# AaltoML/free-hunch

Measured on AMD Instinct MI355X. Metric: images/sec (256x256, num_steps=30, FH-Heun), higher is better.
Workload: dtype f32 UNet (convolutions: exact 3-way bf16 split on the bf16 MFMA, fp32 accuracy) + f64 covariance/CG; 1 GPU; FFHQ-256 arch, gaussian_blur, FH low-rank covariance (dct_diagonal), num_steps=30 heun, batch=8 per GPU; lockstep_groups_per_gpu=2, unet_backend=hip, net_calls_per_image=59

## Files before the change

### free-hunch_amd/_lib.py

```python
from __future__ import annotations

import ctypes as C
import os

import torch

_HERE = os.path.dirname(os.path.abspath(__file__))
LIB_PATH = os.path.join(_HERE, "libfh_hip.so")

c_dp = C.c_void_p


class FhProblem(C.Structure):
    _fields_ = [("op", C.c_int32), ("use_dct", C.c_int32), ("planes", C.c_int32), ("stride", C.c_int32),
                ("ntaps", C.c_int32), ("m", C.c_int32), ("ldm", C.c_int32), ("halo", C.c_int32),
                ("d", C.c_int64), ("sigma_y2", C.c_double),
                ("tap_dy", c_dp), ("tap_dx", c_dp), ("tap_w", c_dp), ("mask", c_dp),
                ("D", c_dp), ("r", c_dp), ("B", c_dp), ("M", c_dp),
                ("ntaps2", C.c_int32), ("halo2", C.c_int32), ("cg_scipy", C.c_int32), ("fold_sym", C.c_int32),
                ("tap2_dy", c_dp), ("tap2_dx", c_dp), ("tap2_w", c_dp),
                ("fold_fwd_w", c_dp), ("fold_fwd_h", c_dp), ("fold_inv_w", c_dp), ("fold_inv_h", c_dp)]


FH_MAX_BATCH = 16
# ... 12 lines not shown


class FhGnEpilogue(C.Structure):
    _fields_ = [("partial", c_dp), ("x", c_dp), ("tab", c_dp), ("mode", C.c_int32), ("act", C.c_int32), ("in_amax", c_dp)]


class FhCgInfo(C.Structure):
    _fields_ = [("niter", C.c_int32), ("optimal", C.c_int32), ("residual_norm", C.c_double),
                ("b_norm", C.c_double)]


_SIGS = {
    "fh_version": ([], C.c_int),
    "fh_context_create": ([C.POINTER(C.c_void_p), C.c_int, C.c_int, C.c_int], C.c_int),
    "fh_context_destroy": ([C.c_void_p], C.c_int),
    "fh_context_set_exclusive": ([C.c_void_p, C.c_int], C.c_int),
    "fh_context_status": ([C.c_void_p, C.c_void_p], C.c_int),
    "fh_debug_read_stamps": ([C.c_void_p, C.POINTER(C.c_ulonglong), C.c_int, C.c_void_p], C.c_int),
    "fh_dct2d": ([C.c_void_p, c_dp, c_dp, C.c_int, C.c_int, C.c_void_p], C.c_int),
    "fh_dct_moments_u8": ([C.c_void_p, c_dp, C.c_int, c_dp, c_dp, c_dp, C.c_void_p], C.c_int),
    "fh_rep_apply": ([C.c_void_p, c_dp, c_dp, c_dp, c_dp, C.c_int, c_dp, c_dp, C.c_int64, C.c_int, C.c_void_p], C.c_int),
    "fh_rep_apply_batched": ([C.c_void_p, C.POINTER(FhBatch), C.c_int, c_dp, c_dp, C.c_int64, C.c_int, C.c_void_p], C.c_int),
    "fh_rep_invert": ([C.c_void_p, c_dp, c_dp, c_dp, C.c_double, c_dp, c_dp, c_dp, C.c_int, C.c_int64, C.c_int,
                       C.c_void_p], C.c_int),
    "fh_space_prep": ([C.c_void_p, c_dp, C.c_double, c_dp, c_dp, c_dp, C.c_int64, C.c_void_p], C.c_int),
    "fh_dot": ([C.c_void_p, c_dp, c_dp, c_dp, C.c_int, C.c_int64, C.c_void_p], C.c_int),
    "fh_space_commit": ([C.c_void_p, c_dp, c_dp, C.c_double, C.c_double, C.c_double, c_dp, c_dp, c_dp, c_dp, c_dp,
                         c_dp, c_dp, c_dp, C.c_int, C.c_int64, C.c_void_p], C.c_int),
    "fh_space_commit_dev": ([C.c_void_p, c_dp, c_dp, c_dp, C.c_double, c_dp, c_dp, c_dp, c_dp, c_dp, c_dp, c_dp, c_dp,
                             c_dp, C.c_int, C.c_int, c_dp, C.c_int, C.c_int, C.c_int, C.c_int64, C.c_void_p], C.c_int),
    "fh_cov_time_update": ([C.c_void_p, C.POINTER(FhCovState), c_dp, c_dp, C.c_double, C.c_double, C.c_double, C.c_int,
                            c_dp, c_dp, c_dp, c_dp, C.c_void_p], C.c_int),
    "fh_cov_space_update": ([C.c_void_p, C.POINTER(FhCovState), c_dp, c_dp, C.c_double, c_dp, c_dp, C.c_void_p], C.c_int),
    "fh_cov_time_update_batched": ([C.c_void_p, C.c_int, C.POINTER(FhCovState), c_dp, c_dp, C.c_double, C.c_double, C.c_double,
                                    c_dp, c_dp, c_dp, C.c_void_p], C.c_int),
    "fh_cov_space_update_batched": ([C.c_void_p, C.c_int, C.POINTER(FhCovState), c_dp, c_dp, C.c_double, c_dp, c_dp, c_dp,
                                     C.c_void_p], C.c_int),
    "fh_woodbury_inner": ([C.c_void_p, c_dp, C.c_int, c_dp, C.c_int, c_dp, C.c_int, C.c_int, C.c_void_p], C.c_int),
    "fh_axpby": ([C.c_double, c_dp, C.c_double, c_dp, c_dp, C.c_int64, C.c_void_p], C.c_int),
    "fh_read_scalars": ([C.c_void_p, c_dp, C.POINTER(C.c_double), C.c_int, C.c_void_p], C.c_int),
    "fh_conv_circ": ([C.c_void_p, c_dp, c_dp, c_dp, c_dp, c_dp, C.c_int, C.c_int, C.c_int, C.c_int, C.c_int,
                      C.c_void_p], C.c_int),
    "fh_channel_mix": ([C.c_void_p, c_dp, c_dp, c_dp, C.c_int, C.c_int, C.c_void_p], C.c_int),
    "fh_amm": ([C.c_void_p, C.POINTER(FhProblem), c_dp, c_dp, C.c_void_p], C.c_int),
    "fh_dense_matvec_scratch_doubles": ([C.c_int, C.c_int64], C.c_int64),
    "fh_dense_matvec": ([c_dp, c_dp, c_dp, c_dp, C.c_int, C.c_int64, C.c_int, C.c_double, C.c_double, C.c_void_p], C.c_int),
    "fh_dense_rank2": ([c_dp, c_dp, C.c_int, C.c_int64, c_dp, c_dp, c_dp, c_dp, c_dp, c_dp, C.c_double, C.c_double,
                        C.c_void_p], C.c_int),
    "fh_conv2d_nhwc": ([c_dp, c_dp, c_dp, c_dp, c_dp, c_dp] + [C.c_int] * 10 + [C.c_void_p], C.c_int),
    "fh_conv2d_x6_nhwc": ([c_dp, c_dp, c_dp, c_dp, c_dp, c_dp] + [C.c_int] * 10 + [C.c_void_p], C.c_int),
    "fh_conv2d_x6_nhwc_gn": ([c_dp, c_dp, c_dp, c_dp, c_dp, c_dp] + [C.c_int] * 10 + [C.POINTER(FhGnEpilogue), C.c_void_p],
                             C.c_int),
    "fh_conv2d_x6_gn_chunks": ([C.c_int] * 10, C.c_int),
    "fh_groupnorm_finalize": ([c_dp, c_dp, C.c_int, C.c_int, C.c_double, C.c_int, C.c_void_p], C.c_int),
    "fh_groupnorm_bwd_table": ([c_dp, c_dp, c_dp, c_dp, c_dp, C.c_int, c_dp, C.c_int, C.c_int, C.c_void_p], C.c_int),
    "fh_groupnorm_bwd_apply": ([c_dp] * 8 + [C.c_int, c_dp] + [C.c_int] * 5 + [C.c_void_p], C.c_int),
    "fh_groupnorm_bwd_sums": ([c_dp] * 7 + [C.c_int, c_dp, c_dp] + [C.c_int] * 4 + [C.c_void_p], C.c_int),
    "fh_groupnorm_bwd_apply_ex": ([c_dp] * 8 + [C.c_int, c_dp, c_dp, c_dp, c_dp] + [C.c_int] * 5 + [c_dp, C.c_void_p], C.c_int),
    "fh_conv2d_splitk": ([C.c_int] * 7, C.c_int),
    "fh_unet_set_precision": ([C.c_int], C.c_int),
    "fh_unet_get_precision": ([], C.c_int),
    "fh_absmax_f32": ([c_dp, C.c_int64, c_dp, C.c_void_p], C.c_int),
    "fh_groupnorm_table": ([c_dp, c_dp, c_dp, c_dp, c_dp, C.c_int, c_dp, C.c_int, C.c_int, C.c_void_p], C.c_int),
    "fh_conv2d_x6_norm_supported": ([C.c_int] * 5, C.c_int),
    "fh_conv2d_x6_norm_nhwc": ([c_dp, c_dp, C.c_int, c_dp, c_dp, c_dp, c_dp] + [C.c_int] * 5 + [C.c_void_p], C.c_int),
    "fh_conv2d_x6_norm_nhwc_gn": ([c_dp, c_dp, C.c_int, c_dp, c_dp, c_dp, c_dp] + [C.c_int] * 5
                                  + [C.POINTER(FhGnEpilogue), C.c_void_p], C.c_int),
    "fh_conv3x3_thin_nhwc": ([c_dp, c_dp, c_dp, c_dp] + [C.c_int] * 5 + [C.c_void_p], C.c_int),
    "fh_conv3x3_wino_nhwc": ([c_dp, c_dp, c_dp, c_dp, c_dp] + [C.c_int] * 5 + [C.c_void_p], C.c_int),
    "fh_bgemm_f32": ([c_dp, c_dp, c_dp] + [C.c_int] * 10 + [C.c_int64] * 6 + [C.c_float, C.c_void_p], C.c_int),
    "fh_groupnorm_scratch_doubles": ([C.c_int, C.c_int], C.c_int64),
    "fh_groupnorm_stats": ([c_dp, c_dp, c_dp, C.c_int, C.c_int, C.c_int, C.c_void_p], C.c_int),
    "fh_groupnorm_apply": ([c_dp] * 6 + [C.c_int, c_dp, C.c_int, C.c_int, C.c_int, C.c_int, C.c_void_p], C.c_int),
    "fh_groupnorm_bwd": ([c_dp] * 7 + [C.c_int, c_dp, c_dp, c_dp] + [C.c_int] * 5 + [C.c_void_p], C.c_int),
    "fh_attention_supported": ([C.c_int] * 3, C.c_int),
    "fh_attention_fwd": ([c_dp, c_dp, c_dp] + [C.c_int] * 5 + [C.c_void_p], C.c_int),
    "fh_attention_bwd": ([c_dp] * 6 + [C.c_int] * 5 + [C.c_void_p], C.c_int),
    "fh_softmax_rows": ([c_dp, C.c_int64, C.c_int, C.c_void_p], C.c_int),
    "fh_softmax_bwd_rows": ([c_dp, c_dp, C.c_int64, C.c_int, C.c_void_p], C.c_int),
    "fh_resample2x": ([c_dp, c_dp] + [C.c_int] * 5 + [C.c_void_p], C.c_int),
    "fh_concat_channels": ([c_dp, c_dp, c_dp, C.c_int64, C.c_int, C.c_int, C.c_int, C.c_void_p], C.c_int),
    "fh_layout_nchw_nhwc": ([c_dp, c_dp, C.c_int, C.c_int, C.c_int64, C.c_int, C.c_int, C.c_void_p], C.c_int),
    "fh_add_f32": ([c_dp, c_dp, c_dp, C.c_int64, C.c_void_p], C.c_int),
    "fh_metrics_scratch_doubles": ([C.c_int] * 4, C.c_int64),
    "fh_metrics_u8": ([c_dp, c_dp, C.c_int, C.c_int, C.c_int, C.c_int, c_dp, c_dp, c_dp, C.c_void_p], C.c_int),
    "fh_lpips_prep_u8": ([c_dp, c_dp, c_dp, c_dp, C.c_int, C.c_int, C.c_int, C.c_void_p], C.c_int),
    "fh_relu_f32": ([c_dp, C.c_int64, C.c_void_p], C.c_int),
    "fh_relu_maxpool2_nhwc": ([c_dp, c_dp, C.c_int, C.c_int, C.c_int, C.c_int, C.c_void_p], C.c_int),
    "fh_lpips_tap_scratch_doubles": ([C.c_int], C.c_int64),
    "fh_lpips_tap": ([c_dp, c_dp, C.c_int, C.c_int, C.c_int, C.c_int, c_dp, c_dp, C.c_int, C.c_void_p], C.c_int),
    "fh_cg_solve_batched": ([C.c_void_p, C.POINTER(FhProblem), C.POINTER(FhBatch), c_dp, c_dp, C.POINTER(C.c_double),
                             C.c_double, C.c_int, C.POINTER(FhCgInfo), C.c_void_p], C.c_int),
    "fh_cg_solve": ([C.c_void_p, C.POINTER(FhProblem), c_dp, c_dp, C.c_double, C.c_double, C.c_int,
                     C.POINTER(FhCgInfo), C.c_void_p], C.c_int),
}

_lib = None


class FhError(RuntimeError):
    pass


def load():
    global _lib
    if _lib is None:
# ... 102 lines not shown
```

### free-hunch_amd/csrc/fh_unet.hip

```cpp
#include "fh_common.h"
#include <stdlib.h>

typedef float float16_t __attribute__((ext_vector_type(16)));

namespace {

constexpr int kBK = 32;
constexpr int kLd = kBK + 4;

struct ConvArgs {
  const float* in;
  const float* w;
  const float* bias;
  const float* res;
  float* out;
  int N, H, W, Cin, Cout, KH, KW, pad, stride, Ho, Wo;
  int ksplit;
  float* ws;
};

__device__ __forceinline__ void xcd_tile(int& tile_m, int& tile_n) {
  const unsigned gx = gridDim.x, gy = gridDim.y;
  const unsigned total = gx * gy;
  unsigned lin = blockIdx.y * gx + blockIdx.x;
// ... 412 lines not shown
    float tb[5] = {0.f, 0.f, 0.f, 0.f, 0.f};
    if (gn && a.gn_mode == 1) {
#pragma unroll
      for (int q = 0; q < 5; ++q) tb[q] = a.gn_tab[((int64_t)gn_n * 5 + q) * a.Cout + co];
    }
#pragma unroll
    for (int i = 0; i < MI; ++i) {
#pragma unroll
      for (int r = 0; r < 16; ++r) {
        const int64_t row = m0 + wm + i * 32 + (r & 3) + 8 * (r >> 2) + 4 * lh;
        if (row < M) {
          float v = acc[i][j][r];
          if (F16 && NP == 2) v = v * ssc.inv_in * ssc.winv;
          v += bv;
          if (a.res != nullptr && a.ksplit == 1) v += a.res[row * a.Cout + co];
          dst[row * a.Cout + co] = v;
          if (gn) gn_accum(a, gsum[j], v, row, co, tb);
        }
      }
    }
  }
  if (gn) {
    const int tiles_per_img = (int)(((int64_t)a.Ho * a.Wo) / BM);
    gn_reduce<NI, WM, WN, BN>(a, gsum, gred, gn_n, (tile_m % tiles_per_img) * (int)gridDim.y + tile_n, n0);
  }
}

template <int SEGW, bool NORM = false, int BM = 128, int NP = 3, int GL = 0, bool F16 = false>
__global__ __launch_bounds__(4 * BM, 4) void k_conv_x6r(ConvArgsX a) {
  constexpr int MI = 2, NI = 1, WN = 4, T = 4 * BM;
  constexpr int NSEG = BM / SEGW, SP = SEGW + 2;
  constexpr int BN = 128, AR = NSEG * SP;
  constexpr int IA = (AR * 8 + T - 1) / T;
  constexpr int IB = (NP * BN * 4 + T - 1) / T;
  constexpr int NB = GL == 2 ? 3 : (GL ? 2 : 1);
  constexpr int NA = GL == 2 ? 2 : 1;
  static_assert(GL != 2 || (NP * 8 == T / 64), "deep pipeline: one weight DMA per wave and tap");
  constexpr int BLD = GL ? kBK : kXLd;
  constexpr int kAsBytes = NA * NP * AR * kXLd * 2, kBsBytes = NB * NP * BN * BLD * 2;
  constexpr int kGredBytes = (BM / 64) * WN * 32 * NI * 2 * 8;
  __shared__ __align__(16) unsigned char smem[kAsBytes + kBsBytes + kGredBytes];
  __bf16 (*As)[NP][AR][kXLd] = reinterpret_cast<__bf16 (*)[NP][AR][kXLd]>(smem);
  __bf16 (*Bs)[NP][BN][BLD] = reinterpret_cast<__bf16 (*)[NP][BN][BLD]>(smem + kAsBytes);
  double* gred = reinterpret_cast<double*>(smem + kAsBytes + kBsBytes);
  const int tid = threadIdx.x, lane = tid & 63, wave = tid >> 6;
  const int wm = (wave / WN) * (MI * 32), wn = (wave % WN) * (NI * 32);
  const int lr = lane & 31, lh = lane >> 5;
  int tile_m, tile_n;
  xcd_tile(tile_m, tile_n);
  const int64_t m0 = (int64_t)tile_m * BM;
  const int n0 = tile_n * BN;
  const int cpt = a.Cin / kBK;
  const int nchunks = cpt * 9;
  const int pn = (int)(m0 / ((int64_t)a.H * a.W));
  const int rem = (int)(m0 % ((int64_t)a.H * a.W));
  const int py = rem / a.W, px0 = rem % a.W;

  int a_row[IA], a_seg[IA], a_gx[IA];
  bool a_in[IA];
  const int a_c4 = (tid & 7) * 4;
#pragma unroll
  for (int e = 0; e < IA; ++e) {
    const int idx = e * T + tid;
    a_row[e] = idx >> 3;
    a_seg[e] = a_row[e] / SP;
    a_gx[e] = px0 - 1 + a_row[e] % SP;
    a_in[e] = idx < AR * 8 && a_gx[e] >= 0 && a_gx[e] < a.W;
    if (idx >= AR * 8) a_row[e] = -1;
  }
  const int64_t wplane = (int64_t)9 * cpt * a.Cout * kBK;
  const SplitScale ssc = split_scale<NP, F16>(a, wplane);
  int b_pl[IB], b_row[IB];
  bool b_ok[IB];
  const int b_part = (tid & 3) * 8;
#pragma unroll
  for (int e = 0; e < IB; ++e) {
    const int idx = e * T + tid;
    b_pl[e] = idx < NP * BN * 4 ? idx / (BN * 4) : -1;
    b_row[e] = (idx % (BN * 4)) >> 2;
    b_ok[e] = b_pl[e] >= 0 && n0 + b_row[e] < a.Cout;
  }
  float4 ra_reg[IA];
  bool ra_ok[IA];
  float4 tA = make_float4(1.f, 1.f, 1.f, 1.f), tB = make_float4(0.f, 0.f, 0.f, 0.f);
  bf16x8_t rb_reg[IB];
  auto load_a = [&](int cc, int ky) {
    if (NORM) {
      const float* t = a.ab + (int64_t)pn * 2 * a.Cin + cc * kBK + a_c4;
      tA = *reinterpret_cast<const float4*>(t);
      tB = *reinterpret_cast<const float4*>(t + a.Cin);
    }
    const float* base = a.in + (int64_t)pn * a.H * a.W * a.Cin + cc * kBK + a_c4;
#pragma unroll
    for (int e = 0; e < IA; ++e) {
      const int gy = py + a_seg[e] + ky - 1;
      const bool ok = a_in[e] && gy >= 0 && gy < a.H;
      ra_ok[e] = ok;
      if (GL == 2) {
        const float4 v = *reinterpret_cast<const float4*>(base + ((int64_t)(ok ? gy : 0) * a.W + (ok ? a_gx[e] : 0)) * a.Cin);
        ra_reg[e] = v;
      } else {
        ra_reg[e] = ok ? *reinterpret_cast<const float4*>(base + ((int64_t)gy * a.W + a_gx[e]) * a.Cin)
                       : make_float4(0.f, 0.f, 0.f, 0.f);
      }
    }
  };
// ... 127 lines not shown
    int cc, tap;
    for (int rg = 0; rg + 1 < nrg; ++rg) {
      const int c0 = 3 * rg, ab = rg & 1;
      load_a((rg + 1) / 3, (rg + 1) % 3);
      tap_args(c0 + 2, cc, tap);
      issue_b(cc, tap, 2);
      compute(0, 0, ab);
      if (kLoads + 1 == 4)
        FH_WAIT_BARRIER(4);
      else
        FH_WAIT_BARRIER(6);
      tap_args(c0 + 3, cc, tap);
      issue_b(cc, tap, 0);
      compute(1, 1, ab);
      FH_WAIT_BARRIER(1);
      tap_args(c0 + 4, cc, tap);
      issue_b(cc, tap, 1);
      compute(2, 2, ab);
      store_a(ab ^ 1);
      FH_WAIT_BARRIER(1);
    }
    {
      const int c0 = 3 * (nrg - 1), ab = (nrg - 1) & 1;
      tap_args(c0 + 2, cc, tap);
      issue_b(cc, tap, 2);
      compute(0, 0, ab);
      FH_WAIT_BARRIER(1);
      compute(1, 1, ab);
      FH_WAIT_BARRIER(0);
      compute(2, 2, ab);
    }
#undef FH_WAIT_BARRIER
  } else if (GL) {
    load_a(0, 0);
    issue_b(0, 0, 0);
    store_a();
    __syncthreads();
    for (int c = 0; c < nchunks; ++c) {
      const int kx = c % 3, nx = c + 1;
      const bool more = nx < nchunks, new_row = more && (nx % 3 == 0);
      if (more) {
        const int ncc = nx / 9, nky = (nx / 3) % 3, nkx = nx % 3;
        issue_b(ncc, nky * 3 + nkx, nx & 1);
        if (new_row) load_a(ncc, nky);
      }
      compute(kx, c & 1);
      __syncthreads();
      if (new_row) {
        store_a();
        __syncthreads();
      }
    }
  } else {
  load_a(0, 0);
  load_b(0, 0);
  store_a();
  store_b(0);
  __syncthreads();
  for (int c = 0; c < nchunks; ++c) {
    const int kx = c % 3;
    const int nx = c + 1;
    const bool more = nx < nchunks;
    const bool new_row = more && (nx % 3 == 0);
    if (more) {
      const int ncc = nx / 9, nky = (nx / 3) % 3, nkx = nx % 3;
      load_b(ncc, nky * 3 + nkx);
      if (new_row) load_a(ncc, nky);
    }
    {
      compute(kx, 0);
      __syncthreads();
      if (more) {
        store_b(0);
        if (new_row) store_a();
        __syncthreads();
      }
    }
  }
  }
  const int64_t M = (int64_t)a.N * a.Ho * a.Wo;
  const bool gn = a.gn_partial != nullptr;
  GnAcc gsum[NI];
#pragma unroll
  for (int j = 0; j < NI; ++j) {
    gsum[j].s0 = gsum[j].s1 = 0.f;
    const int co = n0 + wn + j * 32 + lr;
    if (co >= a.Cout) continue;
    const float bv = a.bias != nullptr ? a.bias[co] : 0.f;
    float tb[5] = {0.f, 0.f, 0.f, 0.f, 0.f};
    if (gn && a.gn_mode == 1) {
#pragma unroll
      for (int q = 0; q < 5; ++q) tb[q] = a.gn_tab[((int64_t)pn * 5 + q) * a.Cout + co];
    }
#pragma unroll
    for (int i = 0; i < MI; ++i) {
#pragma unroll
      for (int r = 0; r < 16; ++r) {
        const int64_t row = m0 + wm + i * 32 + (r & 3) + 8 * (r >> 2) + 4 * lh;
        if (row < M) {
          float v = acc[i][j][r];
          if (F16 && NP == 2) v = v * ssc.inv_in * ssc.winv;
          v += bv;
          if (a.res != nullptr) v += a.res[row * a.Cout + co];
          a.out[row * a.Cout + co] = v;
          if (gn) gn_accum(a, gsum[j], v, row, co, tb);
        }
      }
    }
  }
  if (gn) gn_reduce<NI, BM / 64, WN, BN>(a, gsum, gred, pn, (rem / BM) * (int)gridDim.y + tile_n, n0);
}

constexpr int kWK = 16;
constexpr int kWLd = kWK + 4;

template <int TB>
__global__ __launch_bounds__(512) void k_conv_wino(ConvArgs a) {
  constexpr int BN = 64;
  __shared__ __align__(16) float Ds[2][2][TB + 2][kWLd];
  __shared__ __align__(16) float Us[2][4][BN][kWLd];
  const int tid = threadIdx.x, lane = tid & 63, wave = tid >> 6;
  constexpr int MI = TB / 128;
  const int wm = (wave >> 1) * (32 * MI), wn = (wave & 1) * 32;
  const int lr = lane & 31, lh = lane >> 5;
  const int Wt = a.W / 2;
  const int64_t Mt = (int64_t)a.N * a.H * Wt;
  const int64_t t0 = (int64_t)blockIdx.x * TB;
  const int n0 = blockIdx.y * BN;
  const int cpt = a.Cin / kWK;
  const int nchunks = 3 * cpt;

  constexpr int NI = (TB + 2) * 8 / 512 + 1;
  int it_y[NI], it_slot[NI], it_q[NI];
  int64_t it_base[NI];
  bool it_ok[NI];
#pragma unroll
  for (int e = 0; e < NI; ++e) {
    const int item = tid + 512 * e;
    const bool has = e < NI - 1 || tid < 16;
    const int ps = item >> 2;
    it_q[e] = (item & 3) * 4;
    it_slot[e] = ps;
    const int64_t tg = t0 + (ps >> 1) - 1;
    it_ok[e] = has && tg >= 0 && tg < Mt;
    it_y[e] = 0;
    it_base[e] = 0;
    if (it_ok[e]) {
      const int n = (int)(tg / ((int64_t)a.H * Wt));
      const int rem = (int)(tg % ((int64_t)a.H * Wt));
      it_y[e] = rem / Wt;
      const int x = (rem % Wt) * 2 + (ps & 1);
      it_base[e] = (((int64_t)n * a.H) * a.W + x) * a.Cin + it_q[e];
    }
    if (!has) it_slot[e] = -1;
  }
  const int ub_pos[2] = {tid >> 8, 2 + (tid >> 8)};
  const int ub_co = (tid >> 2) & 63, ub_q = (tid & 3) * 4;
// ... 567 lines not shown
  const int C4 = (Ca + Cb) / 4, Ca4 = Ca / 4, Cb4 = Cb / 4;
  for (int64_t i = (int64_t)blockIdx.x * 256 + threadIdx.x; i < P * C4; i += (int64_t)gridDim.x * 256) {
    const int c4 = (int)(i % C4);
    const int64_t p = i / C4;
    float4* o = reinterpret_cast<float4*>(out) + i;
    float4* s = c4 < Ca4 ? reinterpret_cast<float4*>(a) + p * Ca4 + c4 : reinterpret_cast<float4*>(b) + p * Cb4 + (c4 - Ca4);
    if (split) *s = *o; else *o = *s;
  }
}

__global__ __launch_bounds__(256) void k_nchw_to_nhwc(const float* __restrict__ in, float* __restrict__ out, int N,
                                                      int C, int64_t P, int Cp) {
  for (int64_t i = (int64_t)blockIdx.x * 256 + threadIdx.x; i < (int64_t)N * P * Cp; i += (int64_t)gridDim.x * 256) {
    const int c = (int)(i % Cp);
    const int64_t p = (i / Cp) % P, n = i / (Cp * P);
    out[i] = c < C ? in[((int64_t)n * C + c) * P + p] : 0.f;
  }
}
__global__ __launch_bounds__(256) void k_nhwc_to_nchw(const float* __restrict__ in, float* __restrict__ out, int N,
                                                      int C, int64_t P, int Cp) {
  for (int64_t i = (int64_t)blockIdx.x * 256 + threadIdx.x; i < (int64_t)N * C * P; i += (int64_t)gridDim.x * 256) {
    const int64_t p = i % P;
    const int c = (int)((i / P) % C);
    const int64_t n = i / (P * C);
    out[i] = in[((int64_t)n * P + p) * Cp + c];
  }
}

__global__ __launch_bounds__(256) void k_add_f32(const float* __restrict__ a, const float* __restrict__ b,
                                                 float* __restrict__ out, int64_t n4) {
  for (int64_t i = (int64_t)blockIdx.x * 256 + threadIdx.x; i < n4; i += (int64_t)gridDim.x * 256) {
    const float4 x = reinterpret_cast<const float4*>(a)[i], y = reinterpret_cast<const float4*>(b)[i];
    reinterpret_cast<float4*>(out)[i] = make_float4(x.x + y.x, x.y + y.y, x.z + y.z, x.w + y.w);
  }
}

inline unsigned grid_for(int64_t work_items, int per_block = 256, int cap = 4096) {
  int64_t b = (work_items + per_block - 1) / per_block;
  return (unsigned)(b < 1 ? 1 : (b > cap ? cap : b));
}

thread_local int g_conv_np = 3;

struct X6Plan {
  bool reuse;
  int bm, bn;
  int segw;
  int gl;
  dim3 grid, block;
  bool norm;
  int gn_bm;
};

X6Plan x6_plan(int ksplit, int N, int H, int W, int , int Cout, int KH, int KW, int pad,
               int stride, bool norm) {
  const int Ho = (H + 2 * pad - KH) / stride + 1, Wo = (W + 2 * pad - KW) / stride + 1;
  const int64_t M = (int64_t)N * Ho * Wo;
  const int nb128 = (Cout + 127) / 128;
  const int64_t b128 = ((M + 127) / 128) * nb128;
  X6Plan p{};
  p.bn = 128, p.norm = norm;
  if (ksplit == 1 && Cout > 64 && b128 >= 384) {
    const bool r3 = KH == 3 && KW == 3 && pad == 1 && stride == 1 && M % 128 == 0;
    const bool big = r3 && M % 256 == 0 && (M / 256) * nb128 >= 256;
    p.reuse = true;
    if (big && W % 256 == 0)
      p.bm = 256, p.segw = 256;
    else if (big && W == 128 && H % 2 == 0)
      p.bm = 256, p.segw = 128;
    else if (big && W == 64 && H % 4 == 0)
      p.bm = 256, p.segw = 64;
    else if (r3 && W % 128 == 0)
      p.bm = 128, p.segw = 128;
    else if (r3 && W == 64 && H % 2 == 0)
      p.bm = 128, p.segw = 64;
    else if (r3 && W == 32 && H % 4 == 0)
      p.bm = 128, p.segw = 32;
    else
      p.reuse = false, p.bm = 128;
    p.gl = p.bm == 256;
  } else if (ksplit > 1 && Cout > 64 && b128 * ksplit >= 256) {
    p.bm = 128;
  } else if (ksplit == 1 && Cout > 64 && ((M + 63) / 64) * nb128 >= 256) {
    p.bm = 64;
  } else {
    p.bm = 64, p.bn = 64;
  }
  p.grid = dim3((unsigned)((M + p.bm - 1) / p.bm), (unsigned)((Cout + p.bn - 1) / p.bn), (unsigned)ksplit);
  p.block = dim3(p.reuse ? 4 * p.bm : (p.bm == 128 ? 512 : 256));
  p.gn_bm = (ksplit == 1 && Cout > 64 && p.bn == 128 && Cout % 32 == 0 && (Ho * Wo) % p.bm == 0) ? p.bm : 0;
  return p;
}

template <int SEGW, bool NORM, int BM, int GL>
void launch_x6r(const X6Plan& p, hipStream_t st, const ConvArgsX& a) {
  switch (g_conv_np) {
    case 1: hipLaunchKernelGGL((k_conv_x6r<SEGW, NORM, BM, 1, GL>), p.grid, p.block, 0, st, a); break;
    case 2: hipLaunchKernelGGL((k_conv_x6r<SEGW, NORM, BM, 2, GL>), p.grid, p.block, 0, st, a); break;
    case 16: hipLaunchKernelGGL((k_conv_x6r<SEGW, NORM, BM, 1, GL, true>), p.grid, p.block, 0, st, a); break;
    case 32: hipLaunchKernelGGL((k_conv_x6r<SEGW, NORM, BM, 2, GL == 1 ? 2 : GL, true>), p.grid, p.block, 0, st, a); break;
    default: hipLaunchKernelGGL((k_conv_x6r<SEGW, NORM, BM, 3, GL>), p.grid, p.block, 0, st, a); break;
  }
}

template <int MI, int NI, int WM, int WN, int MINW>
void launch_x6(const X6Plan& p, hipStream_t st, const ConvArgsX& a) {
  switch (g_conv_np) {
    case 1: hipLaunchKernelGGL((k_conv_x6<MI, NI, WM, WN, MINW, 1>), p.grid, p.block, 0, st, a); break;
    case 2: hipLaunchKernelGGL((k_conv_x6<MI, NI, WM, WN, MINW, 2>), p.grid, p.block, 0, st, a); break;
    case 16: hipLaunchKernelGGL((k_conv_x6<MI, NI, WM, WN, MINW, 1, true>), p.grid, p.block, 0, st, a); break;
    case 32: hipLaunchKernelGGL((k_conv_x6<MI, NI, WM, WN, MINW, 2, true>), p.grid, p.block, 0, st, a); break;
    default: hipLaunchKernelGGL((k_conv_x6<MI, NI, WM, WN, MINW, 3>), p.grid, p.block, 0, st, a); break;
  }
}

constexpr int tile_key(int bm, int w, int gl = 0) { return (bm * 1024 + w) * 2 + gl; }

template <bool NORM>
bool launch_x6r_tile(const X6Plan& p, hipStream_t st, const ConvArgsX& a) {
  switch (tile_key(p.bm, p.segw, p.gl)) {
    case tile_key(256, 256, 1): launch_x6r<256, NORM, 256, 1>(p, st, a); return true;
    case tile_key(256, 128, 1): launch_x6r<128, NORM, 256, 1>(p, st, a); return true;
    case tile_key(256, 64, 1): launch_x6r<64, NORM, 256, 1>(p, st, a); return true;
    case tile_key(128, 128, 0): launch_x6r<128, NORM, 128, 0>(p, st, a); return true;
    case tile_key(128, 64, 0): launch_x6r<64, NORM, 128, 0>(p, st, a); return true;
    case tile_key(128, 32, 0): launch_x6r<32, NORM, 128, 0>(p, st, a); return true;
  }
  return false;
}

bool launch_x6_tile(const X6Plan& p, hipStream_t st, const ConvArgsX& a) {
  switch (tile_key(p.bm, p.bn)) {
    case tile_key(128, 128): launch_x6<2, 1, 2, 4, 4>(p, st, a); return true;
    case tile_key(64, 128): launch_x6<1, 2, 2, 2, 2>(p, st, a); return true;
    case tile_key(64, 64): launch_x6<1, 1, 2, 2, 2>(p, st, a); return true;
  }
  return false;
}

}

extern "C" {

int fh_unet_set_precision(int mode) {
  if (mode < 0 || mode > 4) return FH_EINVAL;
  g_conv_np = mode == 0 ? 3 : (mode == 1 ? 1 : (mode == 2 ? 2 : (mode == 3 ? 16 : 32)));
  return 0;
}

int fh_unet_get_precision(void) {
  return g_conv_np == 3 ? 0 : (g_conv_np == 1 ? 1 : (g_conv_np == 2 ? 2 : (g_conv_np == 16 ? 3 : 4)));
}

int fh_absmax_f32(const float* x, int64_t n, float* out, void* stream) {
  if (!out || n < 0 || (n > 0 && !x) || ((uintptr_t)x & 15)) return FH_EINVAL;
  hipStream_t st = (hipStream_t)stream;
  FH_CHECK(hipMemsetAsync(out, 0, FH_AMAX_SLOTS * sizeof(float), st));
  if (n > 0) {
    const int64_t want = (n / 4 + 255) / 256;
    hipLaunchKernelGGL(k_absmax, dim3((unsigned)(want < 1 ? 1 : (want > 2048 ? 2048 : want))), dim3(256), 0, st, x, n,
                       reinterpret_cast<unsigned*>(out));
  }
  FH_LAUNCH_CHECK();
  return 0;
}

int fh_conv2d_splitk(int N, int Ho, int Wo, int Cin, int Cout, int KH, int KW) {
  const int64_t M = (int64_t)N * Ho * Wo;
  const int64_t blocks = ((M + 63) / 64) * ((Cout + 63) / 64);
  const int nchunks = KH * KW * (Cin / kBK);
  int z = 1;
  constexpr int target = 2048;
  constexpr int zmax = 8;
  while (blocks * z < target && z < zmax && nchunks / (2 * z) >= 6) z *= 2;
  return z;
}

int fh_conv2d_nhwc(const float* in, const float* w, const float* bias, const float* res, float* out, float* ws,
                   int ksplit, int N, int H, int W, int Cin, int Cout, int KH, int KW, int pad, int stride,
// ... 68 lines not shown
  hipStream_t st = (hipStream_t)stream;
  const bool built = !p.reuse ? launch_x6_tile(p, st, a)
                     : p.norm ? launch_x6r_tile<true>(p, st, a)
                              : launch_x6r_tile<false>(p, st, a);
  if (!built) return FH_ESIZE;
  if (ksplit > 1) {
    const int64_t total = (int64_t)N * a.Ho * a.Wo * Cout;
    hipLaunchKernelGGL(k_splitk_reduce, dim3(grid_for(total)), dim3(256), 0, st, (const float*)ws, bias, res, out, total,
                       Cout, ksplit);
  }
  FH_LAUNCH_CHECK();
  return 0;
}

int fh_conv2d_x6_nhwc(const float* in, const void* wx, const float* bias, const float* res, float* out, float* ws,
                      int ksplit, int N, int H, int W, int Cin, int Cout, int KH, int KW, int pad, int stride,
                      void* stream) {
  return conv2d_x6_launch(in, false, nullptr, 0, wx, bias, res, out, ws, ksplit, N, H, W, Cin, Cout, KH, KW, pad, stride,
                          nullptr, stream);
}

int fh_conv2d_x6_nhwc_gn(const float* in, const void* wx, const float* bias, const float* res, float* out, float* ws,
                         int ksplit, int N, int H, int W, int Cin, int Cout, int KH, int KW, int pad, int stride,
                         const fh_gn_epilogue* epi, void* stream) {
  return conv2d_x6_launch(in, false, nullptr, 0, wx, bias, res, out, ws, ksplit, N, H, W, Cin, Cout, KH, KW, pad, stride,
                          epi, stream);
}

__global__ __launch_bounds__(256) void k_gn_table(const float* __restrict__ stats, const float* __restrict__ gamma,
                                                  const float* __restrict__ beta, const float* __restrict__ scale,
                                                  const float* __restrict__ shift, int ss_stride,
                                                  float* __restrict__ table, int C) {
  const int n = blockIdx.x, cg = C / 32;
  for (int c = threadIdx.x; c < C; c += 256) {
    const int64_t si = ((int64_t)n * 32 + c / cg) * 2;
    const float mean = stats[si], rstd = stats[si + 1];
    const float sc = scale != nullptr ? 1.f + scale[(int64_t)n * ss_stride + c] : 1.f;
    const float sh = shift != nullptr ? shift[(int64_t)n * ss_stride + c] : 0.f;
    const float rg = rstd * gamma[c];
    table[((int64_t)n * 2 + 0) * C + c] = rg * sc;
    table[((int64_t)n * 2 + 1) * C + c] = (beta[c] - mean * rg) * sc + sh;
  }
}

int fh_groupnorm_table(const float* stats, const float* gamma, const float* beta, const float* scale, const float* shift,
                       int ss_stride, float* table, int N, int C, void* stream) {
  if (!stats || !gamma || !beta || !table || N < 1 || C % 32 != 0) return FH_EINVAL;
  hipLaunchKernelGGL(k_gn_table, dim3(N), dim3(256), 0, (hipStream_t)stream, stats, gamma, beta, scale, shift, ss_stride,
                     table, C);
  FH_LAUNCH_CHECK();
  return 0;
}

int fh_conv2d_x6_norm_supported(int N, int H, int W, int Cin, int Cout) {
  if (N < 1 || H < 1 || W < 1 || Cin < kBK || Cin % kBK != 0 || Cout < 1) return 0;
  return x6_plan(1, N, H, W, Cin, Cout, 3, 3, 1, 1, true).reuse;
}

int fh_conv2d_x6_norm_nhwc(const float* in, const float* ab_table, int act, const void* wx, const float* bias,
                           const float* res, float* out, int N, int H, int W, int Cin, int Cout, void* stream) {
  return conv2d_x6_launch(in, true, ab_table, act, wx, bias, res, out, nullptr, 1, N, H, W, Cin, Cout, 3, 3, 1, 1, nullptr,
                          stream);
}

int fh_conv2d_x6_norm_nhwc_gn(const float* in, const float* ab_table, int act, const void* wx, const float* bias,
                              const float* res, float* out, int N, int H, int W, int Cin, int Cout, const fh_gn_epilogue* epi,
                              void* stream) {
  return conv2d_x6_launch(in, true, ab_table, act, wx, bias, res, out, nullptr, 1, N, H, W, Cin, Cout, 3, 3, 1, 1, epi,
                          stream);
}

int fh_conv3x3_thin_nhwc(const float* in, const float* w, const float* bias, float* out, int N, int H, int W, int Cin,
                         int Cout, void* stream) {
  if (!in || !w || !out || N < 1 || N > 65535 || H < 1 || W < 1 || Cin < 32 || Cin % 32 != 0 || Cout < 1 || Cout > 8)
    return FH_EINVAL;
  const dim3 grid((W + 15) / 16, (H + 15) / 16, N);
  if (Cout <= 4)
    hipLaunchKernelGGL(k_conv_thin<4>, grid, dim3(256), 0, (hipStream_t)stream, in, w, bias, out, H, W, Cin, Cout);
  else
    hipLaunchKernelGGL(k_conv_thin<8>, grid, dim3(256), 0, (hipStream_t)stream, in, w, bias, out, H, W, Cin, Cout);
  FH_LAUNCH_CHECK();
  return 0;
}

int fh_conv3x3_wino_nhwc(const float* in, const float* wu, const float* bias, const float* res, float* out, int N,
                         int H, int W, int Cin, int Cout, void* stream) {
  if (!in || !wu || !out || N < 1 || H < 1 || W < 2 || (W & 1) || Cin < kWK || Cin % kWK != 0 || Cout < 1)
    return FH_EINVAL;
  ConvArgs a;
  a.in = in, a.w = wu, a.bias = bias, a.res = res, a.out = out;
  a.N = N, a.H = H, a.W = W, a.Cin = Cin, a.Cout = Cout, a.KH = 3, a.KW = 3, a.pad = 1, a.stride = 1;
  a.Ho = H, a.Wo = W, a.ksplit = 1, a.ws = nullptr;
  const int64_t Mt = (int64_t)N * H * (W / 2);
  const int nb = (Cout + 63) / 64;
  if (((Mt + 255) / 256) * nb >= 224)
    hipLaunchKernelGGL(k_conv_wino<256>, dim3((unsigned)((Mt + 255) / 256), nb, 1), dim3(512), 0, (hipStream_t)stream, a);
  else
    hipLaunchKernelGGL(k_conv_wino<128>, dim3((unsigned)((Mt + 127) / 128), nb, 1), dim3(512), 0, (hipStream_t)stream, a);
  FH_LAUNCH_CHECK();
  return 0;
}

int fh_bgemm_f32(const float* A, const float* B, float* C, int M, int N, int K, int lda, int ldb, int ldc, int transA,
                 int transB, int batch, int inner, int64_t sA0, int64_t sA1, int64_t sB0, int64_t sB1, int64_t sC0,
                 int64_t sC1, float alpha, void* stream) {
  if (!A || !B || !C || M < 1 || N < 1 || K < 1 || batch < 1 || inner < 1) return FH_EINVAL;
// ... 204 lines not shown
```

### include/fh_hip.h

```cpp
#ifndef FH_HIP_H
#define FH_HIP_H

#include <stdint.h>

#ifdef __cplusplus
extern "C" {
#endif

#define FH_EINVAL (-1)
#define FH_ESYNC (-3)
#define FH_ESIZE (-2)
#define FH_MAX_COLS 256

typedef struct fh_context fh_context;

int fh_version(void);
int fh_context_create(fh_context** out, int S, int planes_max, int m_cap);
int fh_context_destroy(fh_context* ctx);
int fh_context_set_exclusive(fh_context* ctx, int exclusive);
int fh_context_status(fh_context* ctx, void* stream);
int fh_debug_read_stamps(fh_context* ctx, unsigned long long* out_host, int count, void* stream);

int fh_dct2d(fh_context* ctx, const double* in, double* out, int planes, int inverse, void* stream);

// ... 95 lines not shown
  int32_t nimg;
  int32_t pad;
  const double* D[FH_MAX_BATCH];
  const double* r[FH_MAX_BATCH];
  const double* B[FH_MAX_BATCH];
  const double* M[FH_MAX_BATCH];
  const double* mask[FH_MAX_BATCH];
} fh_batch;

typedef struct fh_cg_info {
  int32_t niter;
  int32_t optimal;
  double residual_norm;
  double b_norm;
} fh_cg_info;

int fh_rep_apply_batched(fh_context* ctx, const fh_batch* per, int ldm, const double* z, double* out, int64_t d, int m,
                         void* stream);

int fh_amm(fh_context* ctx, const fh_problem* p, const double* u, double* out, void* stream);
int fh_cg_solve(fh_context* ctx, const fh_problem* p, const double* b, double* x, double rtol, double atol,
                int maxiter, fh_cg_info* info_host, void* stream);
int fh_cg_solve_batched(fh_context* ctx, const fh_problem* shared, const fh_batch* per, const double* b, double* x,
                        const double* rtol_host, double atol, int maxiter, fh_cg_info* info_host, void* stream);


int fh_conv2d_nhwc(const float* in, const float* w, const float* bias, const float* res, float* out, float* ws,
                   int ksplit, int N, int H, int W, int Cin, int Cout, int KH, int KW, int pad, int stride,
                   void* stream);
int fh_unet_set_precision(int mode);
int fh_unet_get_precision(void);
#define FH_AMAX_SLOTS 16
int fh_absmax_f32(const float* x, int64_t n, float* out, void* stream);
int fh_conv2d_splitk(int N, int Ho, int Wo, int Cin, int Cout, int KH, int KW);

int fh_conv2d_x6_nhwc(const float* in, const void* wx, const float* bias, const float* res, float* out, float* ws,
                      int ksplit, int N, int H, int W, int Cin, int Cout, int KH, int KW, int pad, int stride,
                      void* stream);

int fh_groupnorm_table(const float* stats, const float* gamma, const float* beta, const float* scale, const float* shift,
                       int ss_stride, float* table, int N, int C, void* stream);
int fh_conv2d_x6_norm_supported(int N, int H, int W, int Cin, int Cout);
int fh_conv2d_x6_norm_nhwc(const float* in, const float* ab_table, int act, const void* wx, const float* bias,
                           const float* res, float* out, int N, int H, int W, int Cin, int Cout, void* stream);

typedef struct fh_gn_epilogue {
  double* partial;
  const float* x;
  const float* tab;
  int32_t mode, act;
  const float* in_amax;
} fh_gn_epilogue;
int fh_conv2d_x6_gn_chunks(int ksplit, int N, int H, int W, int Cin, int Cout, int KH, int KW, int pad, int stride);
int fh_conv2d_x6_nhwc_gn(const float* in, const void* wx, const float* bias, const float* res, float* out, float* ws,
                         int ksplit, int N, int H, int W, int Cin, int Cout, int KH, int KW, int pad, int stride,
                         const fh_gn_epilogue* epi, void* stream);
int fh_conv2d_x6_norm_nhwc_gn(const float* in, const float* ab_table, int act, const void* wx, const float* bias,
                              const float* res, float* out, int N, int H, int W, int Cin, int Cout, const fh_gn_epilogue* epi,
                              void* stream);
int fh_groupnorm_finalize(const double* partial, float* out, int N, int chunks, double count, int mode, void* stream);
int fh_groupnorm_bwd_table(const float* stats, const float* gamma, const float* beta, const float* scale, const float* shift,
                           int ss_stride, float* table, int N, int C, void* stream);
int fh_groupnorm_bwd_apply(const float* x, const float* dy, const float* stats, const float* sums, const float* gamma,
                           const float* beta, const float* scale, const float* shift, int ss_stride, float* dx, int N, int P,
                           int C, int act, int accumulate, void* stream);
int fh_groupnorm_bwd_sums(const float* x, const float* dy, const float* stats, const float* gamma, const float* beta,
                          const float* scale, const float* shift, int ss_stride, float* sums, double* scratch, int N, int P,
                          int C, int act, void* stream);
int fh_groupnorm_bwd_apply_ex(const float* x, const float* dy, const float* stats, const float* sums, const float* gamma,
                              const float* beta, const float* scale, const float* shift, int ss_stride, const float* acc_src,
                              const float* add2, float* dx, float* dx2, int csplit, int N, int P, int C, int act, float* amax2,
                              void* stream);

int fh_conv3x3_thin_nhwc(const float* in, const float* w, const float* bias, float* out, int N, int H, int W, int Cin,
                         int Cout, void* stream);

int fh_conv3x3_wino_nhwc(const float* in, const float* wu, const float* bias, const float* res, float* out, int N,
                         int H, int W, int Cin, int Cout, void* stream);

int fh_bgemm_f32(const float* A, const float* B, float* C, int M, int N, int K, int lda, int ldb, int ldc, int transA,
                 int transB, int batch, int inner, int64_t sA0, int64_t sA1, int64_t sB0, int64_t sB1, int64_t sC0,
                 int64_t sC1, float alpha, void* stream);

int64_t fh_groupnorm_scratch_doubles(int N, int P);
int fh_groupnorm_stats(const float* x, float* stats, double* scratch, int N, int P, int C, void* stream);
int fh_groupnorm_apply(const float* x, const float* stats, const float* gamma, const float* beta, const float* scale,
                       const float* shift, int ss_stride, float* y, int N, int P, int C, int act, void* stream);
int fh_groupnorm_bwd(const float* x, const float* dy, const float* stats, const float* gamma, const float* beta,
                     const float* scale, const float* shift, int ss_stride, float* sums, double* scratch, float* dx, int N,
                     int P, int C, int act, int accumulate, void* stream);

int fh_softmax_rows(float* s, int64_t rows, int T, void* stream);
int fh_softmax_bwd_rows(const float* p, float* dp, int64_t rows, int T, void* stream);

int fh_attention_supported(int T, int C, int heads);
int fh_attention_fwd(const float* qkv, float* out, float* lse, int N, int T, int C, int heads, int new_order, void* stream);
int fh_attention_bwd(const float* qkv, const float* out, const float* dout, const float* lse, float* dsum, float* dqkv, int N,
                     int T, int C, int heads, int new_order, void* stream);

int fh_resample2x(const float* in, float* out, int N, int Hs, int Ws, int C, int mode, void* stream);

int fh_concat_channels(float* a, float* b, float* out, int64_t P, int Ca, int Cb, int split, void* stream);

int fh_layout_nchw_nhwc(const float* in, float* out, int N, int C, int64_t P, int Cp, int to_nhwc, void* stream);

int fh_add_f32(const float* a, const float* b, float* out, int64_t n, void* stream);
// ... 24 lines not shown
```

Baseline: 2.307 images/s.

## Extend row-reuse x6 conv kernel to split-K launches with workspace partial outputs

Lets the row-reuse implicit-GEMM conv kernel run with split-K. Each z-slice processes its own chunk range aligned to kernel rows and writes partial sums to the workspace, leaving bias and residual to the existing reduction. The planner now picks this path for 3x3 stride-1 convs with small widths (64/32/16) when split boundaries align, and adds a 16-wide tile. This brings input-row reuse to low-resolution layers that previously used the generic split-K path, at the cost of more template instantiations and stricter alignment conditions.

```diff
diff --git a/free-hunch_amd/_lib.py b/free-hunch_amd/_lib.py
--- a/free-hunch_amd/_lib.py
+++ b/free-hunch_amd/_lib.py
@@ -88,6 +88,7 @@
     "fh_conv2d_x6_nhwc_gn": ([c_dp, c_dp, c_dp, c_dp, c_dp, c_dp] + [C.c_int] * 10 + [C.POINTER(FhGnEpilogue), C.c_void_p],
                              C.c_int),
     "fh_conv2d_x6_gn_chunks": ([C.c_int] * 10, C.c_int),
+    "fh_conv2d_x6_row_reuse": ([C.c_int] * 10, C.c_int),
     "fh_groupnorm_finalize": ([c_dp, c_dp, C.c_int, C.c_int, C.c_double, C.c_int, C.c_void_p], C.c_int),
     "fh_groupnorm_bwd_table": ([c_dp, c_dp, c_dp, c_dp, c_dp, C.c_int, c_dp, C.c_int, C.c_int, C.c_void_p], C.c_int),
     "fh_groupnorm_bwd_apply": ([c_dp] * 8 + [C.c_int, c_dp] + [C.c_int] * 5 + [C.c_void_p], C.c_int),
diff --git a/free-hunch_amd/csrc/fh_unet.hip b/free-hunch_amd/csrc/fh_unet.hip
--- a/free-hunch_amd/csrc/fh_unet.hip
+++ b/free-hunch_amd/csrc/fh_unet.hip
@@ -488,6 +488,8 @@
   const int n0 = tile_n * BN;
   const int cpt = a.Cin / kBK;
   const int nchunks = cpt * 9;
+  const int c_begin = GL ? 0 : (int)((int64_t)nchunks * blockIdx.z / a.ksplit);
+  const int c_end = GL ? nchunks : (int)((int64_t)nchunks * (blockIdx.z + 1) / a.ksplit);
   const int pn = (int)(m0 / ((int64_t)a.H * a.W));
   const int rem = (int)(m0 % ((int64_t)a.H * a.W));
   const int py = rem / a.W, px0 = rem % a.W;
@@ -721,15 +723,15 @@
       }
     }
   } else {
-  load_a(0, 0);
-  load_b(0, 0);
+  load_a(c_begin / 9, (c_begin / 3) % 3);
+  load_b(c_begin / 9, c_begin % 9);
   store_a();
   store_b(0);
   __syncthreads();
-  for (int c = 0; c < nchunks; ++c) {
+  for (int c = c_begin; c < c_end; ++c) {
     const int kx = c % 3;
     const int nx = c + 1;
-    const bool more = nx < nchunks;
+    const bool more = nx < c_end;
     const bool new_row = more && (nx % 3 == 0);
     if (more) {
       const int ncc = nx / 9, nky = (nx / 3) % 3, nkx = nx % 3;
@@ -749,13 +751,16 @@
   }
   const int64_t M = (int64_t)a.N * a.Ho * a.Wo;
   const bool gn = a.gn_partial != nullptr;
+  const bool whole = a.ksplit == 1;
+  float* dst = whole ? a.out : a.ws + (int64_t)blockIdx.z * M * a.Cout;
+  const float* res = whole ? a.res : nullptr;
   GnAcc gsum[NI];
 #pragma unroll
   for (int j = 0; j < NI; ++j) {
     gsum[j].s0 = gsum[j].s1 = 0.f;
     const int co = n0 + wn + j * 32 + lr;
     if (co >= a.Cout) continue;
-    const float bv = a.bias != nullptr ? a.bias[co] : 0.f;
+    const float bv = (a.bias != nullptr && whole) ? a.bias[co] : 0.f;
     float tb[5] = {0.f, 0.f, 0.f, 0.f, 0.f};
     if (gn && a.gn_mode == 1) {
 #pragma unroll
@@ -770,8 +775,8 @@
           float v = acc[i][j][r];
           if (F16 && NP == 2) v = v * ssc.inv_in * ssc.winv;
           v += bv;
-          if (a.res != nullptr) v += a.res[row * a.Cout + co];
-          a.out[row * a.Cout + co] = v;
+          if (res != nullptr) v += res[row * a.Cout + co];
+          dst[row * a.Cout + co] = v;
           if (gn) gn_accum(a, gsum[j], v, row, co, tb);
         }
       }
@@ -1445,8 +1450,7 @@
   int gn_bm;
 };
 
-X6Plan x6_plan(int ksplit, int N, int H, int W, int , int Cout, int KH, int KW, int pad,
-               int stride, bool norm) {
+X6Plan x6_plan(int ksplit, int N, int H, int W, int Cin, int Cout, int KH, int KW, int pad, int stride, bool norm) {
   const int Ho = (H + 2 * pad - KH) / stride + 1, Wo = (W + 2 * pad - KW) / stride + 1;
   const int64_t M = (int64_t)N * Ho * Wo;
   const int nb128 = (Cout + 127) / 128;
@@ -1474,6 +1478,11 @@
     p.gl = p.bm == 256;
   } else if (ksplit > 1 && Cout > 64 && b128 * ksplit >= 256) {
     p.bm = 128;
+    const int nchunks = 9 * (Cin / kBK);
+    bool aligned = KH == 3 && KW == 3 && pad == 1 && stride == 1 && M % 128 == 0 && ((int64_t)H * W) % 128 == 0;
+    for (int z = 1; z < ksplit && aligned; ++z) aligned = ((int64_t)nchunks * z / ksplit) % 3 == 0;
+    const int segw = (W == 64 && H % 2 == 0) ? 64 : (W == 32 && H % 4 == 0) ? 32 : (W == 16 && H % 8 == 0) ? 16 : 0;
+    if (aligned && segw) p.reuse = true, p.segw = segw;
   } else if (ksplit == 1 && Cout > 64 && ((M + 63) / 64) * nb128 >= 256) {
     p.bm = 64;
   } else {
@@ -1518,6 +1527,12 @@
     case tile_key(128, 128, 0): launch_x6r<128, NORM, 128, 0>(p, st, a); return true;
     case tile_key(128, 64, 0): launch_x6r<64, NORM, 128, 0>(p, st, a); return true;
     case tile_key(128, 32, 0): launch_x6r<32, NORM, 128, 0>(p, st, a); return true;
+    case tile_key(128, 16, 0):
+      if constexpr (!NORM) {
+        launch_x6r<16, false, 128, 0>(p, st, a);
+        return true;
+      }
+      return false;
   }
   return false;
 }
@@ -1692,6 +1707,11 @@
   return 0;
 }
 
+int fh_conv2d_x6_row_reuse(int ksplit, int N, int H, int W, int Cin, int Cout, int KH, int KW, int pad, int stride) {
+  if (ksplit < 1 || ksplit > 32 || N < 1 || H < 1 || W < 1 || Cin < kBK || Cin % kBK != 0 || Cout < 1 || stride < 1) return 0;
+  return x6_plan(ksplit, N, H, W, Cin, Cout, KH, KW, pad, stride, false).reuse;
+}
+
 int fh_conv2d_x6_norm_supported(int N, int H, int W, int Cin, int Cout) {
   if (N < 1 || H < 1 || W < 1 || Cin < kBK || Cin % kBK != 0 || Cout < 1) return 0;
   return x6_plan(1, N, H, W, Cin, Cout, 3, 3, 1, 1, true).reuse;
diff --git a/include/fh_hip.h b/include/fh_hip.h
--- a/include/fh_hip.h
+++ b/include/fh_hip.h
@@ -171,6 +171,7 @@
   const float* in_amax;
 } fh_gn_epilogue;
 int fh_conv2d_x6_gn_chunks(int ksplit, int N, int H, int W, int Cin, int Cout, int KH, int KW, int pad, int stride);
+int fh_conv2d_x6_row_reuse(int ksplit, int N, int H, int W, int Cin, int Cout, int KH, int KW, int pad, int stride);
 int fh_conv2d_x6_nhwc_gn(const float* in, const void* wx, const float* bias, const float* res, float* out, float* ws,
                          int ksplit, int N, int H, int W, int Cin, int Cout, int KH, int KW, int pad, int stride,
                          const fh_gn_epilogue* epi, void* stream);
```

New measurement: 2.358 images/s (median of 6 runs). 2.2% higher.
